# uzh-rpg/rampvo

Measured on AMD Instinct MI355X. Metric: keyframes/sec (BA iters/sec) SingleScale 640x480; ATE vs reference, higher is better.
Workload: dtype f16 (features, MFMA inputs; f32 accumulate, hidden state, BA, geometry: default.yaml MIXED_PRECISION); 1 GPU; BASELINE configs[1]: SingleScale 640x480, 96 patches/frame, default.yaml windows, 2 BA iters/keyframe, steady-state sliding window; edges=38880, edges_end=38880, keyframes_in_window=184, prime_frames=70, clock_warm=480 untimed steady-state steps (0.43 s) before the 5 warm-up steps, frame_pipelining=True, pipeline_gate=signal word stored by the gru launch, full=False

## Files before the change

include/ramp_hip.h:

```cpp
#ifndef RAMP_HIP_H
#define RAMP_HIP_H

#include <stddef.h>
#include <stdint.h>

#ifdef __cplusplus
extern "C" {
#endif

#define RAMP_OK 0
#define RAMP_EINVAL -1
#define RAMP_ELAUNCH -2
#define RAMP_EWORKSPACE -3
#define RAMP_EUNSUPPORTED -4

#define RAMP_F32 0
#define RAMP_F16 1

#define RAMP_CORR_MFMA32 0x40
#define RAMP_CORR_X2 0x80

#define RAMP_NCHW 0
#define RAMP_NHWC 1
#define RAMP_NHWC32 2

const char *ramp_version(void);


int ramp_patchify_fwd(const void *net, const float *coords, void *out, int n, int C, int H,
                      int W, int M, int radius, int bilinear, int dtype, int layout,
                      int out_layout, void *stream);

int ramp_frame_gather(const void *fmap, const void *imap, const float *image, const float *coords, void *gmap,
                      void *imap_p, float *patches, float *clr, unsigned char *colors, int M, int h, int w, int H,
                      int W, int CF, int CI, int dtype, void *stream);

typedef struct {
  const void *fmap;
  int H2, W2;
  float coord_div;
} ramp_corr_level;

int ramp_corr_fwd(const void *fmap1, const ramp_corr_level *levels_host, int nlevels,
                  const float *coords, const int64_t *ii, const int64_t *jj, void *out, int E,
                  int N1, int N2, int C, int P, int radius, int dtype, int layout,
                  void *stream);

int ramp_corr_fwd_ordered(const void *fmap1, const ramp_corr_level *levels_host, int nlevels,
                          const float *coords, const int64_t *ii, const int64_t *jj,
                          const int32_t *order, void *out, int out_row_elems, long mod_ii, long mod_jj, int E,
                          int N1, int N2, int C, int P, int radius, int dtype, int layout, void *stream);

int ramp_pyramid_pack(const void *fmap, void *level1, void *level4, int H, int W, int C, int dtype,
                      void *stream);
int ramp_corr_kplane(void);

size_t ramp_event_stack_workspace_bytes(int bins, int H, int W);
int ramp_event_stack(const int32_t *x, const int32_t *y, const int8_t *p, int N, int bins, int H, int W,
                     int8_t *out_i8, float *out_f32, void *ws, size_t ws_bytes, void *stream);

int ramp_depth_median_fill(const float *patches_src, int F, int M, int P, float *patches_dst, void *stream);
int ramp_depth_median(const float *patches_src, int F, int M, int P, float *out, void *stream);

size_t ramp_event_topk_workspace_bytes(int H, int W);
int ramp_event_topk(const float *events, int bins, int H, int W, int k, int nms_kernel_size, float *coords,
                    int64_t *indices, void *ws, size_t ws_bytes, void *stream);

int ramp_se3_exp(const float *a, float *X, int n, void *stream);
int ramp_se3_log(const float *X, float *a, int n, void *stream);
int ramp_se3_inv(const float *X, float *Y, int n, void *stream);
int ramp_se3_mul(const float *X, const float *Y, float *Z, int n, void *stream);
int ramp_se3_act4(const float *X, const float *p, float *q, int n, void *stream);
int ramp_se3_adj(const float *X, const float *a, float *b, int n, void *stream);
int ramp_se3_adjT(const float *X, const float *a, float *b, int n, void *stream);

int ramp_transform(const float *poses, const float *patches, const float *intrinsics,
                   const int64_t *ii, const int64_t *jj, const int64_t *kk, float *out, int E,
                   int P, int tonly, void *stream);

int ramp_reproject(const float *poses, const float *patches, const float *intrinsics,
                   const int64_t *ii, const int64_t *jj, const int64_t *kk, float *out, int E,
                   int P, void *stream);

int ramp_point_cloud(const float *poses, const float *patches, const float *intrinsics,
                     const int64_t *ix, float *out, int m, int P, void *stream);

int ramp_motionmag(const float *poses, const float *patches, const float *intrinsics,
                   const int64_t *ii, const int64_t *jj, const int64_t *kk, const int32_t *order,
                   const int32_t *seg, const int64_t *ukeys, const int32_t *ngroups, int64_t key_ij,
                   int64_t key_ji, float beta, float *out2, int P, void *stream);

int ramp_motion_model(float *poses, int n, float damping, void *stream);

int ramp_frame_begin(float *poses, int n, int motion, float damping, int64_t *tstamps, int64_t counter,
                     int64_t *index_map, int64_t index_val, float *intrinsics, int copy_k, void *stream);

int ramp_frame_commit(float *poses, int n, int motion, float damping, int64_t *tstamps, int64_t counter,
                      int64_t *index_map, int64_t index_val, float *intrinsics, int copy_k, float *patches_state,
                      int median_frames, int M, int P, float *patches_new, int n_copy, const void *const *src_host,
                      void *const *dst_host, const long *bytes_host, const float *median_dev, void *stream);

int ramp_multi_copy(const void *const *src_host, void *const *dst_host, const long *bytes_host, int n,
                    void *stream);
int ramp_shift_rows(void *const *base_host, const long *row_bytes_host, const int *mod_host, int n, int k,
                    int nrows, void *stream);

size_t ramp_group_by_workspace_bytes(int E);
int ramp_group_by(const int64_t *keys, int E, int64_t key_bound, int32_t *order, int32_t *gid,
                  int32_t *seg_start, int64_t *ukeys, int32_t *ngroups, void *ws,
                  size_t ws_bytes, void *stream);

size_t ramp_neighbors_workspace_bytes(int E);
int ramp_neighbors(const int64_t *kk, const int64_t *jj, int64_t *ix, int64_t *jx, int E,
                   int64_t kk_bound, int64_t jj_bound, void *ws, size_t ws_bytes,
                   void *stream);

int ramp_segment_softmax_sum(const void *fx, const void *gx, const int32_t *order,
                             const int32_t *seg_start, const int32_t *ngroups, void *y, int E,
                             int C, int max_groups, int dtype, void *stream);

size_t ramp_ba_workspace_bytes(int E, int n_poses, int n_patches, int t0, int t1);
int ramp_ba_forward(float *poses, float *patches, const float *intrinsics, const float *target,
                    const float *weight, const float *lmbda, const int64_t *ii,
                    const int64_t *jj, const int64_t *kk, int E, int P, int n_poses,
                    int n_patches, int t0, int t1, int iterations, void *ws, size_t ws_bytes,
                    int32_t *info, void *stream);

size_t ramp_ba_planned_workspace_bytes(int E, int n_poses, int n_patches, int t0, int t1,
                                       int max_patches, int max_pairs);
int ramp_ba_forward_planned(float *poses, float *patches, const float *intrinsics, const float *target,
                            const float *weight, const float *lmbda, const int64_t *ii,
                            const int64_t *jj, const int64_t *kk, int E, int P, int n_poses,
                            int n_patches, int t0, int t1, int iterations, const int32_t *order_k,
                            const int32_t *seg_k, const int32_t *ngroups_k, const int64_t *ukeys_k,
                            int max_patches, const int32_t *order_p, const int32_t *seg_p,
                            const int32_t *ngroups_p, int max_pairs, void *ws, size_t ws_bytes,
                            int32_t *info, void *stream);

size_t ramp_group_by_small_workspace_bytes(int E, int K);
int ramp_group_by_small(const int64_t *a, const int64_t *b, int64_t mul, int64_t sub, int K, int E,
                        int32_t *order, int32_t *gid, int32_t *seg_start, int64_t *ukeys,
                        int32_t *ngroups, int max_groups, void *ws, size_t ws_bytes, void *stream);

int ramp_neighbors_from_groups(const int32_t *order, const int32_t *seg_start, const int32_t *ngroups,
                               const int64_t *jj, int64_t *ix, int64_t *jx, int32_t *kj_order, int E,
                               int max_groups, void *stream);

int ramp_any_nonzero(const float *a, long na, const float *b, long nb, int32_t *flags, void *stream);
int ramp_any_nonzero_blocks(const float *a, long na, const float *b, long nb, int32_t *blockflags, void *stream);
int ramp_any_nonzero_blocks_clear(const float *a, long na, const float *b, long nb, int32_t *blockflags, void *clear,
                                  long clear_bytes, void *stream);

int ramp_lstm_superstate_tiled(const float *ev, const float *im, float *h_ev, float *c_ev, float *h_im,
                               float *c_im, float *ss, const float *wfrag, const int32_t *flags, int HW,
                               int has_state, int has_ss, void *stream);
int ramp_lstm_superstate_blocks(const float *ev, const float *im, float *h_ev, float *c_ev, float *h_im,
                                float *c_im, float *ss, const float *wfrag, const int32_t *blockflags, int nblk, int HW,
                                int has_state, int has_ss, void *stream);

int ramp_ms_lstm_superstate(const float *ev, const float *im, const float *const *weights_host,
                            float *state, int H, int W, int scale, int has_state, int use_im,
                            void *stream);

int ramp_ms_lstm_superstate_mfma(const float *ev, const float *im, const float *wfrag, const float *wsmall, float *state,
                                 void *state16, int H, int W, int scale, int has_state, int use_im, void *stream);

int ramp_conv2d_nhwc(const void *x, const void *wpk, const float *bias, const float *pre_scale,
                     const float *pre_shift, const void *res, void *y, float *stats, int H, int W,
                     int Cin, int Cout, int KH, int KW, int stride, int relu, float out_scale,
                     int dtype, void *stream);

typedef struct ramp_conv_job {
  const void *x, *wpk;
  const float *bias, *pre_scale, *pre_shift;
  const void *res;
  void *y;
  float *stats;
  int32_t Cout, relu;
  float out_scale;
  float act_scale, w_scale;
  void *acc_out;
  const void *acc_in;
  float in_count, in_eps;
  const void *x2;
  int32_t c0;
  const void *skip;
  const void *acc_skip;
  float skip_count, skip_eps;
  int32_t skip_relu;
  void *mat;
} ramp_conv_job;
#define RAMP_IN_ACC_R 8
int ramp_conv2d_nhwc_multi(const ramp_conv_job *jobs, int njobs, int H, int W, int Cin, int KH, int stride,
                           int dtype, void *stream);

#define RAMP_IN_F32 0x10
#define RAMP_CONV_DIRECT 0x20
#define RAMP_CONV_FP8 0x40

#define RAMP_CONV_X3 0x80

int ramp_conv2d_stats_blocks(int H, int W, int Cin, int Cout, int KH, int stride, int dtype);

int ramp_in_stats_finalize(const float *partial, int nblk, int C, float count, float eps, float *scale,
                           float *shift, void *stream);

int ramp_norm_add_relu_f16_acc(const void *y, const void *acc_y, float count_y, float eps_y, const void *skip,
                               const void *acc_skip, float count_skip, float eps_skip, void *out, long n, int C,
                               int skip_relu, void *stream);
int ramp_in_acc_finalize(const void *acc, int C, float count, float eps, float *scale, float *shift, void *stream);

int ramp_affine_relu(const float *x, const float *s, const float *h, float *out, long n, int C,
                     void *stream);

int ramp_affine_relu_f16(const void *x, const float *s, const float *h, void *out, long n, int C,
                         void *stream);
int ramp_norm_add_relu_f16(const void *y, const float *sy, const float *hy, const void *skip,
                           const float *ss, const float *hs, void *out, long n, int C, int skip_relu,
                           void *stream);

int ramp_norm_add_relu(const float *y, const float *sy, const float *hy, const float *skip,
                       const float *ss, const float *hs, float *out, long n, int C, void *stream);

int ramp_upd_row_fuse(const float *A, const int64_t *idxA, const void *B, const void *C, const int64_t *idxB,
                      const int32_t *idxB32, long modB, const int64_t *idxC, const int32_t *idxC32,
                      const float *ln_w, const float *ln_b, float eps, int relu, float *out_f32,
                      void *out_t, int E, int dtype, void *stream);
int ramp_upd_gather_mask(const float *X, const int64_t *idx, void *out, int E, int dtype, void *stream);
int ramp_upd_gated(const float *X, const void *G, const void *R, const float *ln_w, const float *ln_b,
                   float eps, float *out_f32, void *out_t, void *out_relu_t, int E, int dtype,
                   void *stream);
int ramp_upd_heads(const void *hw, const float *coords, float *target, float *weight, float *delta,
                   int E, int P, float wd, float ht, int dtype, void *stream);
int ramp_upd_segment_softmax(const void *fg, const int32_t *order, const int32_t *seg_start,
                             const int32_t *ngroups, void *y, int max_groups, int dtype, void *stream);

int ramp_graph_edit_host(const int64_t *ii, const int64_t *jj, const int64_t *kk, const int64_t *rows_in, int E,
                         int M, int k_remove, int n_after, int removal_window, int64_t *out, int cap,
                         int64_t *ranges );

int ramp_upd_gru(const float *x32, const void *add_t, const int32_t *add_idx, const float *pre_w, const float *pre_b,
                 float pre_eps, const void *const *wp_host, const float *const *bias_host, const float *ln_w,
                 const float *ln_b, float eps, float *out32, void *relu_t, int E, void *stream);
int ramp_upd_gru_heads(const float *x32, const void *add_t, const int32_t *add_idx, const float *pre_w, const float *pre_b,
                       float pre_eps, const void *const *wp_host, const float *const *bias_host, const float *ln_w,
                       const float *ln_b, float eps, float *out32, const void *heads_w, const float *heads_b,
                       const float *coords, float *target, float *weight, int E, int P, float wd, float ht, void *stream);
size_t ramp_upd_mlp_lds_bytes(void);

int ramp_upd_nbr(const float *net_in, const int64_t *idx, const void *wa, const float *ba, const void *wb,
                 const float *bb, float *net_out, void *out_t, int E, void *stream);

int ramp_upd_corr_mlp(const void *corr, int corr_k, const void *w1, const float *b1, const void *w2, const float *b2,
                      const void *w3, const float *b3, const float *ln_w, const float *ln_b, float ln_eps,
                      const float *net, const int64_t *net_map, const void *inp, const int64_t *inp_idx, long inp_mod,
                      const float *norm_w, const float *norm_b, float norm_eps, float *net_out, int E, void *stream);

int ramp_upd_heads_linear(const void *relu_t, const void *heads_w, const float *heads_b, const float *coords,
                          float *target, float *weight, int E, int P, float wd, float ht, void *stream);

int ramp_upd_fg(const float *x32, const void *add_t, const int32_t *add_idx, float *x32_out, const void *wf,
                const float *bf, const void *wg, const float *bg, void *fg, int E, void *stream);

int ramp_upd_linear(const void *x, const void *w_packed, const float *bias, void *y, int rows, const int32_t *rows_dev,
                    void *stream);

size_t ramp_upd_softagg_frag_rows(int E, int max_groups);
int ramp_upd_softagg(const float *x32, const void *add_t, const int32_t *add_idx, const int32_t *order,
                     const int32_t *gid, const void *wf, const float *bf, const void *wg, const float *bg, float *frag,
                     int E, void *stream);
int ramp_upd_softagg_finish(const float *frag, const int32_t *seg_start, const int32_t *ngroups, const void *wh,
                            const float *bh, void *hy, int max_groups, void *stream);

int ramp_x3_corr_mlp(const float *corr, int corr_k, const void *w1, const float *b1, const void *w2, const float *b2,
                     const void *w3, const float *b3, const float *ln_w, const float *ln_b, float ln_eps, const float *net,
                     const int64_t *net_map, const float *inp, const int64_t *inp_idx, long inp_mod, const float *norm_w,
                     const float *norm_b, float norm_eps, float *net_out, int E, void *stream);
int ramp_x3_nbr(const float *net_in, const int64_t *idx, const void *wa, const float *ba, const void *wb, const float *bb,
                float *net_out, int E, void *stream);
// ... 122 lines not shown
```

rampvo_amd/_lib.py:

```python
import ctypes
import os
import subprocess

import torch

_HERE = os.path.dirname(os.path.abspath(__file__))
CSRC = os.path.join(_HERE, "csrc")
LIB_PATH = os.environ.get("RAMP_HIP_LIB") or os.path.join(CSRC, "libramp_hip.so")

RAMP_F32, RAMP_F16 = 0, 1
RAMP_EUNSUPPORTED = -4
RAMP_CONV_FP8 = 0x40
RAMP_IN_F32, RAMP_CONV_DIRECT, RAMP_CORR_MFMA32, RAMP_CORR_X2 = 0x10, 0x20, 0x40, 0x80
RAMP_CONV_X3 = 0x80
RAMP_NCHW, RAMP_NHWC, RAMP_NHWC32 = 0, 1, 2
KPLANE = 32


def kplane(dtype):
    import torch
    return KPLANE if dtype == torch.float16 else KPLANE // 2


def corr_f32_mode():
    import os
    try:
        m = int(os.environ.get("RAMP_CORR_F32_MFMA", "2"))
    except ValueError:
        m = 2
    return m if m in (0, 1, 2) else 2

_ERR = {-1: "RAMP_EINVAL (bad argument)", -2: "RAMP_ELAUNCH (HIP launch/runtime error)",
        -3: "RAMP_EWORKSPACE (workspace too small)", -4: "RAMP_EUNSUPPORTED (size/shape not supported)"}

c_p, c_i, c_i64, c_sz, c_f = ctypes.c_void_p, ctypes.c_int, ctypes.c_int64, ctypes.c_size_t, ctypes.c_float


class CorrLevel(ctypes.Structure):
    _fields_ = [("fmap", c_p), ("H2", c_i), ("W2", c_i), ("coord_div", c_f)]


SIGNATURES = {
    "ramp_version": (ctypes.c_char_p, []),
    "ramp_corr_kplane": (c_i, []),
    "ramp_patchify_fwd": (c_i, [c_p, c_p, c_p] + [c_i] * 10 + [c_p]),
    "ramp_frame_gather": (c_i, [c_p] * 9 + [c_i] * 8 + [c_p]),
    "ramp_corr_fwd": (c_i, [c_p, ctypes.POINTER(CorrLevel), c_i, c_p, c_p, c_p, c_p] + [c_i] * 8 + [c_p]),
    "ramp_ms_lstm_superstate": (c_i, [c_p, c_p, ctypes.POINTER(c_p), c_p, c_i, c_i, c_i, c_i, c_i, c_p]),
    "ramp_ms_lstm_superstate_mfma": (c_i, [c_p] * 6 + [c_i] * 5 + [c_p]),
    "ramp_conv2d_stats_blocks": (c_i, [c_i] * 7),
    "ramp_graph_edit_host": (c_i, [c_p, c_p, c_p, c_p, c_i, c_i, c_i, c_i, c_i, c_p, c_i, c_p]),
    "ramp_event_stack_workspace_bytes": (c_sz, [c_i, c_i, c_i]),
    "ramp_event_stack": (c_i, [c_p, c_p, c_p, c_i, c_i, c_i, c_i, c_p, c_p, c_p, c_sz, c_p]),
    "ramp_depth_median_fill": (c_i, [c_p, c_i, c_i, c_i, c_p, c_p]),
    "ramp_depth_median": (c_i, [c_p, c_i, c_i, c_i, c_p, c_p]),
    "ramp_event_topk_workspace_bytes": (c_sz, [c_i, c_i]),
    "ramp_event_topk": (c_i, [c_p, c_i, c_i, c_i, c_i, c_i, c_p, c_p, c_p, c_sz, c_p]),
    "ramp_pyramid_pack": (c_i, [c_p, c_p, c_p, c_i, c_i, c_i, c_i, c_p]),
    "ramp_corr_fwd_ordered": (c_i, [c_p, ctypes.POINTER(CorrLevel), c_i, c_p, c_p, c_p, c_p, c_p, c_i, ctypes.c_long,
                                    ctypes.c_long] + [c_i] * 8 + [c_p]),
    "ramp_se3_exp": (c_i, [c_p, c_p, c_i, c_p]),
    "ramp_se3_log": (c_i, [c_p, c_p, c_i, c_p]),
    "ramp_se3_inv": (c_i, [c_p, c_p, c_i, c_p]),
    "ramp_se3_mul": (c_i, [c_p, c_p, c_p, c_i, c_p]),
    "ramp_se3_act4": (c_i, [c_p, c_p, c_p, c_i, c_p]),
    "ramp_se3_adj": (c_i, [c_p, c_p, c_p, c_i, c_p]),
    "ramp_se3_adjT": (c_i, [c_p, c_p, c_p, c_i, c_p]),
    "ramp_transform": (c_i, [c_p] * 7 + [c_i, c_i, c_i, c_p]),
    "ramp_reproject": (c_i, [c_p] * 7 + [c_i, c_i, c_p]),
    "ramp_point_cloud": (c_i, [c_p] * 5 + [c_i, c_i, c_p]),
    "ramp_multi_copy": (c_i, [c_p, c_p, c_p, c_i, c_p]),
    "ramp_shift_rows": (c_i, [c_p, c_p, c_p, c_i, c_i, c_i, c_p]),
    "ramp_motionmag": (c_i, [c_p] * 10 + [c_i64, c_i64, c_f, c_p, c_i, c_p]),
    "ramp_motion_model": (c_i, [c_p, c_i, c_f, c_p]),
    "ramp_frame_commit": (c_i, [c_p, c_i, c_i, c_f, c_p, c_i64, c_p, c_i64, c_p, c_i, c_p, c_i, c_i, c_i, c_p, c_i,
                                ctypes.POINTER(c_p), ctypes.POINTER(c_p), ctypes.POINTER(ctypes.c_long), c_p, c_p]),
    "ramp_frame_begin": (c_i, [c_p, c_i, c_i, c_f, c_p, c_i64, c_p, c_i64, c_p, c_i, c_p]),
    "ramp_group_by_workspace_bytes": (c_sz, [c_i]),
    "ramp_group_by": (c_i, [c_p, c_i, c_i64, c_p, c_p, c_p, c_p, c_p, c_p, c_sz, c_p]),
    "ramp_neighbors_workspace_bytes": (c_sz, [c_i]),
    "ramp_neighbors": (c_i, [c_p, c_p, c_p, c_p, c_i, c_i64, c_i64, c_p, c_sz, c_p]),
    "ramp_segment_softmax_sum": (c_i, [c_p] * 6 + [c_i, c_i, c_i, c_i, c_p]),
    "ramp_ba_workspace_bytes": (c_sz, [c_i] * 5),
    "ramp_ba_forward": (c_i, [c_p] * 9 + [c_i] * 7 + [c_p, c_sz, c_p, c_p]),
    "ramp_ba_planned_workspace_bytes": (c_sz, [c_i] * 7),
    "ramp_ba_forward_planned": (c_i, [c_p] * 9 + [c_i] * 7 + [c_p] * 4 + [c_i] + [c_p] * 3 + [c_i, c_p, c_sz, c_p, c_p]),
    "ramp_group_by_small_workspace_bytes": (c_sz, [c_i, c_i]),
    "ramp_group_by_small": (c_i, [c_p, c_p, c_i64, c_i64, c_i, c_i, c_p, c_p, c_p, c_p, c_p, c_i, c_p, c_sz, c_p]),
    "ramp_neighbors_from_groups": (c_i, [c_p] * 7 + [c_i, c_i, c_p]),
    "ramp_any_nonzero": (c_i, [c_p, ctypes.c_long, c_p, ctypes.c_long, c_p, c_p]),
    "ramp_lstm_superstate_tiled": (c_i, [c_p] * 9 + [c_i, c_i, c_i, c_p]),
    "ramp_lstm_superstate_blocks": (c_i, [c_p] * 9 + [c_i, c_i, c_i, c_i, c_p]),
    "ramp_any_nonzero_blocks": (c_i, [c_p, ctypes.c_long, c_p, ctypes.c_long, c_p, c_p]),
    "ramp_any_nonzero_blocks_clear": (c_i, [c_p, ctypes.c_long, c_p, ctypes.c_long, c_p, c_p, ctypes.c_long, c_p]),
    "ramp_conv2d_nhwc": (c_i, [c_p] * 8 + [c_i] * 8 + [c_f, c_i, c_p]),
    "ramp_in_stats_finalize": (c_i, [c_p, c_i, c_i, c_f, c_f, c_p, c_p, c_p]),
    "ramp_affine_relu": (c_i, [c_p, c_p, c_p, c_p, ctypes.c_long, c_i, c_p]),
    "ramp_norm_add_relu": (c_i, [c_p] * 7 + [ctypes.c_long, c_i, c_p]),
    "ramp_affine_relu_f16": (c_i, [c_p, c_p, c_p, c_p, ctypes.c_long, c_i, c_p]),
    "ramp_norm_add_relu_f16": (c_i, [c_p] * 7 + [ctypes.c_long, c_i, c_i, c_p]),
    "ramp_norm_add_relu_f16_acc": (c_i, [c_p, c_p, c_f, c_f, c_p, c_p, c_f, c_f, c_p, ctypes.c_long, c_i, c_i, c_p]),
    "ramp_in_acc_finalize": (c_i, [c_p, c_i, c_f, c_f, c_p, c_p, c_p]),
    "ramp_conv2d_nhwc_multi": (c_i, [c_p, c_i, c_i, c_i, c_i, c_i, c_i, c_i, c_p]),
    "ramp_upd_row_fuse": (c_i, [c_p] * 6 + [ctypes.c_long, c_p, c_p, c_p, c_p, c_f, c_i, c_p, c_p, c_i, c_i, c_p]),
    "ramp_upd_gather_mask": (c_i, [c_p, c_p, c_p, c_i, c_i, c_p]),
    "ramp_upd_gated": (c_i, [c_p] * 5 + [c_f, c_p, c_p, c_p, c_i, c_i, c_p]),
    "ramp_upd_heads": (c_i, [c_p] * 5 + [c_i, c_i, c_f, c_f, c_i, c_p]),
    "ramp_upd_segment_softmax": (c_i, [c_p] * 5 + [c_i, c_i, c_p]),
    "ramp_upd_corr_mlp": (c_i, [c_p, c_i, c_p, c_p, c_p, c_p, c_p, c_p, c_p, c_p, c_f, c_p, c_p, c_p, c_p, ctypes.c_long,
                                c_p, c_p, c_f, c_p, c_i, c_p]),
    "ramp_upd_heads_linear": (c_i, [c_p, c_p, c_p, c_p, c_p, c_p, c_i, c_i, c_f, c_f, c_p]),
    "ramp_upd_fg": (c_i, [c_p] * 9 + [c_i, c_p]),
    "ramp_upd_gru": (c_i, [c_p, c_p, c_p, c_p, c_p, c_f, ctypes.POINTER(c_p), ctypes.POINTER(c_p), c_p, c_p, c_f, c_p,
                           c_p, c_i, c_p]),
    "ramp_upd_gru_heads": (c_i, [c_p, c_p, c_p, c_p, c_p, c_f, ctypes.POINTER(c_p), ctypes.POINTER(c_p), c_p, c_p, c_f, c_p,
                                 c_p, c_p, c_p, c_p, c_p, c_i, c_i, c_f, c_f, c_p]),
    "ramp_upd_mlp_lds_bytes": (c_sz, []),
    "ramp_upd_nbr": (c_i, [c_p] * 8 + [c_i, c_p]),
    "ramp_upd_linear": (c_i, [c_p, c_p, c_p, c_p, c_i, c_p, c_p]),
    "ramp_upd_softagg_frag_rows": (c_sz, [c_i, c_i]),
    "ramp_upd_softagg": (c_i, [c_p] * 10 + [c_i, c_p]),
    "ramp_upd_softagg_finish": (c_i, [c_p] * 6 + [c_i, c_p]),
    "ramp_x3_corr_mlp": (c_i, [c_p, c_i, c_p, c_p, c_p, c_p, c_p, c_p, c_p, c_p, c_f, c_p, c_p, c_p, c_p, ctypes.c_long,
                               c_p, c_p, c_f, c_p, c_i, c_p]),
    "ramp_x3_nbr": (c_i, [c_p] * 7 + [c_i, c_p]),
    "ramp_x3_fg": (c_i, [c_p] * 9 + [c_i, c_p]),
    "ramp_x3_segment_softmax": (c_i, [c_p] * 5 + [c_i, c_p]),
    "ramp_x3_linear": (c_i, [c_p, c_p, c_p, c_p, c_i, c_p, c_p]),
    "ramp_x3_gru": (c_i, [c_p, c_p, c_p, c_p, c_p, c_p, c_p, c_f, ctypes.POINTER(c_p), ctypes.POINTER(c_p), c_p, c_p, c_f,
                          c_p, c_p, c_i, c_p, c_p, c_p, c_p, c_p, c_i, c_f, c_f, c_p]),
    "ramp_track_sizeof": (c_sz, []),
    "ramp_track_plan_workspace_bytes": (c_sz, [c_i, c_i, c_i]),
    "ramp_track_ba_workspace_bytes": (c_sz, [c_i] * 6),
    "ramp_track_plan": (c_i, [c_p, c_i, c_p]),
    "ramp_track_step": (c_i, [c_p, c_i, c_i64, c_i, c_i, c_p, c_p, c_p]),
    "ramp_track_warm": (c_i, [c_p, c_p, c_p]),
    "ramp_stream_delay": (c_i, [c_i, c_p]),
    "ramp_signal_alloc": (c_i, [c_p]),
    "ramp_signal_free": (c_i, [c_p]),
    "ramp_stream_signal": (c_i, [c_p, c_p, ctypes.c_uint32]),
    "ramp_stream_wait_flag": (c_i, [c_p, c_p, ctypes.c_uint32, c_i, c_i, c_p]),
    "ramp_host_device_pointer": (c_i, [c_p, c_p]),
}

_lib = None


def build(force=False, jobs=8):
    cmd = ["make", "-s", "-C", CSRC, "-j%d" % jobs]
    if force:
        cmd.append("-B")
    subprocess.check_call(cmd + ["libramp_hip.so"])
    return LIB_PATH


def register_optional(extra):
    SIGNATURES.update(extra)
    if _lib is not None:
        for name, (res, args) in extra.items():
            fn = getattr(_lib, name)
            fn.restype, fn.argtypes = res, args


def lib():
    global _lib
    if _lib is None:
        if not os.path.exists(LIB_PATH):
            raise RuntimeError(
                "rampvo_amd: %s is missing -- the HIP extension is not built and there is no "
                "CPU fallback (run __graft_entry__.build())" % LIB_PATH)
        l = ctypes.CDLL(LIB_PATH)
        for name, (res, args) in SIGNATURES.items():
            fn = getattr(l, name)
            fn.restype, fn.argtypes = res, args
        if l.ramp_corr_kplane() != KPLANE:
            raise RuntimeError("rampvo_amd: %s packs %d-channel correlation planes, this binding is written for %d "
                               "(rebuild without -DCORR_KPLANE, or set rampvo_amd._lib.KPLANE)" % (LIB_PATH, l.ramp_corr_kplane(), KPLANE))
        _lib = l
    return _lib


def check(rc, what):
    if rc != 0:
        raise RuntimeError("%s failed: %s" % (what, _ERR.get(rc, "status %d" % rc)))


def stream():
    return ctypes.c_void_p(torch._C._cuda_getCurrentRawStream(torch.cuda.current_device()))


def require_cuda(*tensors):
    for t in tensors:
        if t is not None and not t.is_cuda:
            raise RuntimeError("rampvo_amd operators run on the GPU only (got a %s tensor); "
                               "there is no CPU fallback" % t.device)


def dtype_code(t):
    if t.dtype == torch.float32:
        return RAMP_F32
    if t.dtype == torch.float16:
        return RAMP_F16
    raise RuntimeError("unsupported dtype %s (float32 / float16 only)" % t.dtype)


def ptr(t):
    return ctypes.c_void_p(t.data_ptr()) if t is not None else None


_ws_cache = {}
_ws_retired = []
_ws_owner = [None]


class scratch_owner:

    def __init__(self, owner):
        self.owner = owner

    def __enter__(self):
        self.prev, _ws_owner[0] = _ws_owner[0], id(self.owner)

    def __exit__(self, *exc):
        _ws_owner[0] = self.prev


def workspace(nbytes, device, tag="ws"):
    key = (device, torch._C._cuda_getCurrentRawStream(device.index if device.index is not None
                                                      else torch.cuda.current_device()), _ws_owner[0], tag)
    buf = _ws_cache.get(key)
    if buf is None or buf.numel() < nbytes:
        if buf is not None:
            _ws_retired.append(buf)
        buf = torch.empty(max(int(nbytes * 1.25), 1 << 20), dtype=torch.uint8, device=device)
        _ws_cache[key] = buf
    return buf
```

rampvo_amd/csrc/ba.hip:

```cpp
#include "ramp_device.h"
#include <stdlib.h>
#include "ramp_internal.h"

#define BA_REC 32
#define BA_PAIR 160
#define BA_TS 64
#define BA_KB 8

static inline size_t al(size_t x) { return (x + 255) / 256 * 256; }

struct BaEdgeIn {
  const float *poses, *patches, *intr, *target, *weight;
  const int64_t *ii, *jj, *kk;
  int PP, c11, t0, N;
};
__device__ __forceinline__ void ba_edge_compute(const BaEdgeIn &in, int n, float (&r)[BA_REC]) {
  const float fx = in.intr[0], fy = in.intr[1], cx = in.intr[2], cy = in.intr[3];
  int ix = (int)in.ii[n], jx = (int)in.jj[n];
  const long kx = in.kk[n];
  float pi[7], pj[7];
#pragma unroll
  for (int c = 0; c < 7; c++) { pi[c] = in.poses[7 * (size_t)ix + c]; pj[c] = in.poses[7 * (size_t)jx + c]; }
  float Xi[4], Xj[4];
  Xi[0] = (in.patches[((size_t)kx * 3 + 0) * in.PP + in.c11] - cx) / fx;
// ... 629 lines not shown
        for (int k = 0; k < j; k++) x[j] = __builtin_fmaf(-x[k], l[j][k], x[j]);
        x[j] *= li[j];
      }
#pragma unroll
      for (int j = 0; j < 6; j++) A[i * ld + c0 + j] = x[j];
    }
    }
    __syncthreads();
    for (int ii = ty; ii <= m; ii += TG) {
      float ri[6];
#pragma unroll
      for (int k = 0; k < 6; k++) ri[k] = A[(r0 + ii) * ld + c0 + k];
      const int jmax = ii < m - 1 ? ii : m - 1;
      for (int jj = tx; jj <= jmax; jj += TG) {
        const float *rj = A + (r0 + jj) * ld + c0;
        float t = A[(r0 + ii) * ld + r0 + jj];
#pragma unroll
        for (int k = 0; k < 6; k++) t = __builtin_fmaf(-ri[k], rj[k], t);
        A[(r0 + ii) * ld + r0 + jj] = t;
      }
    }
    __syncthreads();
  }
  const bool bad = s_bad != 0;
  if (bad && tid == 0 && info) atomicOr(info, 1);
  if (n6 <= 64) {
    if (tid < 64) {
      float z = tid < n6 ? A[n6 * ld + tid] : 0.0f;
      for (int kb = nb - 1; kb >= 0; kb--) {
        const int c0 = 6 * kb;
        float lk[27], x[6];
#pragma unroll
        for (int q = 0; q < 27; q++) lk[q] = Lk[kb * 28 + q];
#pragma unroll
        for (int j = 0; j < 6; j++) x[j] = __int_as_float(__builtin_amdgcn_readlane(__float_as_int(z), c0 + j));
#pragma unroll
        for (int j = 5; j >= 0; j--) {
#pragma unroll
          for (int k = j + 1; k < 6; k++) x[j] = __builtin_fmaf(-lk[k * (k + 1) / 2 + j], x[k], x[j]);
          x[j] *= lk[21 + j];
        }
        if (tid == 0) {
#pragma unroll
          for (int j = 0; j < 6; j++) xv[c0 + j] = x[j];
        }
        if (tid < c0) {
#pragma unroll
          for (int k = 0; k < 6; k++) z = __builtin_fmaf(-A[(c0 + k) * ld + tid], x[k], z);
        }
      }
    }
    __syncthreads();
  } else
  for (int kb = nb - 1; kb >= 0; kb--) {
    const int c0 = 6 * kb;
    if (tid < 64) {
      float lk[27], x[6];
#pragma unroll
      for (int q = 0; q < 27; q++) lk[q] = Lk[kb * 28 + q];
#pragma unroll
      for (int j = 0; j < 6; j++) x[j] = A[n6 * ld + c0 + j];
#pragma unroll
      for (int j = 5; j >= 0; j--) {
#pragma unroll
        for (int k = j + 1; k < 6; k++) x[j] = __builtin_fmaf(-lk[k * (k + 1) / 2 + j], x[k], x[j]);
        x[j] *= lk[21 + j];
      }
      if (tid == 0) {
#pragma unroll
        for (int j = 0; j < 6; j++) xv[c0 + j] = x[j];
      }
    }
    __syncthreads();
    for (int i = tid; i < c0; i += nt) {
      float t = A[n6 * ld + i];
#pragma unroll
      for (int k = 0; k < 6; k++) t = __builtin_fmaf(-A[(c0 + k) * ld + i], xv[c0 + k], t);
      A[n6 * ld + i] = t;
    }
    __syncthreads();
  }
  __shared__ int s_nf;
  if (tid == 0) s_nf = 0;
  __syncthreads();
  for (int q = tid; q < n6; q += nt)
    if (!(fabsf(xv[q]) <= 3.0e38f)) s_nf = 1;
  __syncthreads();
  const bool drop = bad || s_nf != 0;
  if (!bad && s_nf != 0 && tid == 0 && info) atomicOr(info, 1);
  for (int q = tid; q < n6; q += nt) dX[q] = drop ? 0.0f : xv[q];
}
template <int TG>
__global__ void __launch_bounds__(TG * TG)
    ba_cholb_kernel(const float *__restrict__ S, const float *__restrict__ yv,
                    float *__restrict__ dX, int32_t *__restrict__ info, int n6) {
  extern __shared__ __attribute__((aligned(16))) float sm[];
  const int ld = n6 + 1;
  float *A = sm;
  float *xv = sm + (n6 + 1) * ld;
  float *Lk = xv + n6;
  const int tid = threadIdx.x, nt = TG * TG;
  {
    int r = tid / n6, c = tid - r * n6;
    const int dr = nt / n6, dc = nt - dr * n6;
    for (int q = tid; q < n6 * n6; q += nt) {
      A[r * ld + c] = S[q];
      r += dr; c += dc;
      if (c >= n6) { c -= n6; r++; }
    }
  }
  for (int q = tid; q < n6; q += nt) A[n6 * ld + q] = yv[q];
  ba_cholb_body<TG>(A, xv, Lk, dX, info, n6);
}

__global__ void __launch_bounds__(256)
    ba_retract_kernel(float *__restrict__ poses, float *__restrict__ patches,
                      const float *__restrict__ Erow, const float *__restrict__ Qv,
                      const float *__restrict__ uv, const float *__restrict__ dX,
                      const int64_t *__restrict__ kx, const int32_t *__restrict__ ngroups,
                      int n6, int PP, int t0, int N, int depth_blocks, const int32_t *__restrict__ dyn,
                      int opt_window) {
  if (dyn) {
    const int t1 = dyn[RAMP_DYN_N];
    t0 = max(t1 - opt_window, 1);
    N = min(N, t1 - t0);
  }
  if ((int)blockIdx.x >= depth_blocks) {
    const int i = (blockIdx.x - depth_blocks) * blockDim.x + threadIdx.x;
    if (i >= N) return;
    float *p = poses + 7 * (size_t)(t0 + i);
    float xi[6], to[3] = {p[0], p[1], p[2]}, qo[4] = {p[3], p[4], p[5], p[6]}, tn[3], qn[4];
#pragma unroll
    for (int c = 0; c < 6; c++) xi[c] = dX[6 * i + c];
    fb_retrSE3(xi, to, qo, tn, qn);
    p[0] = tn[0]; p[1] = tn[1]; p[2] = tn[2];
    p[3] = qn[0]; p[4] = qn[1]; p[5] = qn[2]; p[6] = qn[3];
    return;
  }
  const int wave = threadIdx.x / 64, lane = threadIdx.x % 64;
  const int g = blockIdx.x * (blockDim.x / 64) + wave;
  if (g >= *ngroups) return;
  float s = 0.0f;
  for (int a = lane; a < n6; a += 64) s += Erow[(size_t)g * n6 + a] * dX[a];
#pragma unroll
  for (int off = 32; off > 0; off >>= 1) s += __shfl_down(s, off, 64);
  s = __shfl(s, 0, 64);
  const float dz = Qv[g] * (uv[g] - s);
  float *pt = patches + ((size_t)kx[g] * 3 + 2) * PP;
  float dd = pt[0];
  dd = dd + dz;
  dd = (dd > 20) ? 1.0f : dd;
  dd = fmaxf(dd, 1e-4f);
  if (lane < PP) pt[lane] = dd;
}

__global__ void ba_pairkey_kernel(const int64_t *__restrict__ ii, const int64_t *__restrict__ jj,
                                  int64_t *__restrict__ keys, int E, long long np) {
  const int n = blockIdx.x * blockDim.x + threadIdx.x;
  if (n < E) keys[n] = jj[n] * np + ii[n];
}

struct BaWs {
  void *gb; size_t gb_bytes;
  int64_t *pkeys, *kx, *pukeys;
  int32_t *order_k, *seg_k, *order_p, *seg_p, *pair_ij, *counters;
  float *rec, *Erow, *Cv, *uv, *Qv, *pairs, *S_part, *y_part, *S, *yv, *dX;
  int Mu_b, Gp_b, KS, tiles;
};
static size_t ba_carve(void *ws, int E, int n_poses, int n_patches, int N, int own_groups,
                       int max_patches, int max_pairs, BaWs *w) {
  const size_t e = (size_t)(E > 0 ? E : 1);
  const int n6 = 6 * N;
  size_t off = 0;
  char *base = (char *)ws;
  auto take = [&](size_t bytes) { char *p = base ? base + off : nullptr; off += al(bytes); return (void *)p; };
  w->Mu_b = (int)((size_t)n_patches < e ? (size_t)n_patches : e);
  if (max_patches > 0 && max_patches < w->Mu_b) w->Mu_b = max_patches;
  if (w->Mu_b < 1) w->Mu_b = 1;
  const size_t pp = (size_t)n_poses * (size_t)n_poses;
  w->Gp_b = (int)(pp < e ? pp : e);
  if (max_pairs > 0 && max_pairs < w->Gp_b) w->Gp_b = max_pairs;
  if (w->Gp_b < 1) w->Gp_b = 1;
  w->tiles = (n6 + BA_TS - 1) / BA_TS;
  if (w->tiles < 1) w->tiles = 1;
  int ks = 256 / (w->tiles * w->tiles);
  w->KS = ks < 4 ? 4 : (ks > 64 ? 64 : ks);
  w->gb = nullptr; w->gb_bytes = 0;
  w->pkeys = w->kx = w->pukeys = nullptr;
  w->order_k = w->seg_k = w->order_p = w->seg_p = nullptr;
  if (own_groups) {
    w->gb_bytes = ramp_internal_group_by_ws(E);
    w->gb = take(w->gb_bytes);
    w->pkeys = (int64_t *)take(e * 8);
    w->kx = (int64_t *)take(e * 8);
    w->pukeys = (int64_t *)take(e * 8);
    w->order_k = (int32_t *)take(e * 4);
    w->seg_k = (int32_t *)take((e + 1) * 4);
    w->order_p = (int32_t *)take(e * 4);
    w->seg_p = (int32_t *)take((e + 1) * 4);
  }
  w->pair_ij = (int32_t *)take((size_t)w->Gp_b * 8);
  w->counters = (int32_t *)take(64);
  w->rec = (float *)take(e * BA_REC * 4);
  w->Erow = (float *)take((size_t)w->Mu_b * (n6 > 0 ? n6 : 1) * 4);
  w->Cv = (float *)take((size_t)w->Mu_b * 4);
  w->uv = (float *)take((size_t)w->Mu_b * 4);
  w->Qv = (float *)take((size_t)w->Mu_b * 4);
  w->pairs = (float *)take((size_t)w->Gp_b * BA_PAIR * 4);
  w->S_part = (float *)take((size_t)w->KS * (n6 * n6 + 1) * 4);
  w->y_part = (float *)take((size_t)w->KS * (n6 + 1) * 4);
  w->S = (float *)take((size_t)(n6 * n6 + 1) * 4);
  w->yv = (float *)take((size_t)(n6 + 1) * 4);
  w->dX = (float *)take((size_t)(n6 + 1) * 4);
  return off;
}

static int ba_iterate(float *poses, float *patches, const float *intrinsics, const float *target,
                      const float *weight, const float *lmbda, const int64_t *ii, const int64_t *jj,
                      const int64_t *kk, int E, int P, int t0, int t1, int iterations, BaWs &w,
                      const int32_t *order_k, const int32_t *seg_k, const int32_t *nk, const int64_t *kx,
                      const int32_t *order_p, const int32_t *seg_p, const int32_t *np, int32_t *info,
                      hipStream_t st, const int32_t *dyn = nullptr, int opt_window = 0) {
  const int N = t1 - t0, n6 = 6 * N;
  const size_t lds = (size_t)((n6 + 1) * (n6 + 1) + 6 * n6) * sizeof(float);
  const int PP = P * P, c11 = 1 * P + 1;
  if (N > 0 && lds > 64 * 1024) {
    if (hipFuncSetAttribute((const void *)ba_cholb_kernel<32>, hipFuncAttributeMaxDynamicSharedMemorySize, (int)lds) != hipSuccess)
      return RAMP_ELAUNCH;
  }
  const int pthreads = ((n6 + 2 + 63) / 64) * 64;
  if (pthreads > 256) return RAMP_EUNSUPPORTED;
  const int depth_blocks = ramp_cdiv(w.Mu_b, 4);
  const int pose_blocks = N > 0 ? ramp_cdiv(N, 256) : 0;
  BaEdgeIn ein;
  ein.poses = poses; ein.patches = patches; ein.intr = intrinsics; ein.target = target; ein.weight = weight;
  ein.ii = ii; ein.jj = jj; ein.kk = kk; ein.PP = PP; ein.c11 = c11; ein.t0 = t0; ein.N = N;
  const int fuse_edge = 1;
  for (int itr = 0; itr < iterations; itr++) {
    if (N <= 0)
      hipLaunchKernelGGL(ba_edge_kernel, dim3(ramp_cdiv(E, 256)), dim3(256), 0, st, ein, w.rec, E, dyn, opt_window);
    if (N > 0)
      hipLaunchKernelGGL(ba_patch_pair_kernel, dim3(w.Mu_b + w.Gp_b), dim3(256), 0, st, w.Mu_b, w.rec, order_k,
                         seg_k, nk, lmbda, w.Erow, w.Cv, w.uv, w.Qv, n6, order_p, seg_p, np, w.pairs, w.pair_ij, ein,
                         fuse_edge, dyn, opt_window);
    else
      hipLaunchKernelGGL(ba_patch_kernel, dim3(w.Mu_b), dim3(pthreads), 0, st, w.rec, order_k, seg_k, nk,
                         lmbda, w.Erow, w.Cv, w.uv, w.Qv, n6);
    if (N > 0) {
      if (w.tiles == 1 && ramp_cdiv(w.Mu_b, w.KS) <= BA_S1_ROWS)
        hipLaunchKernelGGL(ba_schur1_kernel, dim3(1, 1, w.KS), dim3(256), 0, st, w.Erow, w.Qv, w.uv, nk, w.S_part, w.y_part,
                           n6, w.KS);
      else
        hipLaunchKernelGGL(ba_schur_kernel, dim3(w.tiles, w.tiles, w.KS), dim3(256), 0, st, w.Erow,
                           w.Qv, w.uv, nk, w.S_part, w.y_part, n6, w.KS);
      if (N <= 16)
        hipLaunchKernelGGL(ba_assemble2_kernel, dim3(N, N), dim3(256), 0, st, w.pairs, w.pair_ij, np, w.S_part, w.y_part,
                           w.S, w.yv, n6, w.KS, info);
      else
        hipLaunchKernelGGL(ba_assemble_kernel, dim3(N, ramp_cdiv(6 * n6, 192)), dim3(256), 0, st, w.pairs, w.pair_ij, np,
                           w.S_part, w.y_part, w.S, w.yv, n6, w.KS, info);
      hipLaunchKernelGGL(ba_cholb_kernel<32>, dim3(1), dim3(1024), lds, st, w.S, w.yv, w.dX, info, n6);
    }
    hipLaunchKernelGGL(ba_retract_kernel, dim3(depth_blocks + pose_blocks), dim3(256), 0, st,
                       poses, patches, w.Erow, w.Qv, w.uv, w.dX, kx, nk, n6, PP, t0, N, depth_blocks, dyn, opt_window);
    RAMP_CHECK_LAUNCH();
  }
  return RAMP_OK;
}

static int ba_check_args(int E, int P, int n_poses, int n_patches, int t0, int t1, int iterations) {
  if (E < 0 || P < 2 || n_poses <= 0 || n_patches <= 0 || iterations < 0) return RAMP_EINVAL;
  if (t0 < 0 || t1 < t0 || t1 > n_poses) return RAMP_EINVAL;
  const int n6 = 6 * (t1 - t0);
  if ((size_t)((n6 + 1) * (n6 + 1) + 2 * n6) * sizeof(float) > 160 * 1024) return RAMP_EUNSUPPORTED;
  return RAMP_OK;
}

size_t ramp_i_ba_dyn_ws(int E_cap, int n_poses, int n_patches, int opt_window, int max_patches, int max_pairs) {
  BaWs w;
  return ba_carve(nullptr, E_cap, n_poses, n_patches, opt_window, 0, max_patches, max_pairs, &w);
}
int ramp_i_ba_dyn(float *poses, float *patches, const float *intrinsics, const float *target, const float *weight,
                  const float *lmbda, const int64_t *ii, const int64_t *jj, const int64_t *kk, int E_cap, int P,
                  int n_poses, int n_patches, int opt_window, int iterations, const int32_t *order_k,
                  const int32_t *seg_k, const int32_t *ngroups_k, const int64_t *ukeys_k, int max_patches,
                  const int32_t *order_p, const int32_t *seg_p, const int32_t *ngroups_p, int max_pairs, void *ws,
                  size_t ws_bytes, int32_t *info, const int32_t *dyn, hipStream_t st) {
  if (E_cap <= 0 || opt_window <= 0 || !dyn || !ws) return RAMP_EINVAL;
  int rc = ba_check_args(E_cap, P, n_poses, n_patches, 1, 1 + opt_window, iterations);
  if (rc != RAMP_OK) return rc;
  BaWs w;
  if (ba_carve(ws, E_cap, n_poses, n_patches, opt_window, 0, max_patches, max_pairs, &w) > ws_bytes)
    return RAMP_EWORKSPACE;
  return ba_iterate(poses, patches, intrinsics, target, weight, lmbda, ii, jj, kk, E_cap, P, 1, 1 + opt_window,
                    iterations, w, order_k, seg_k, ngroups_k, ukeys_k, order_p, seg_p, ngroups_p, info, st, dyn,
                    opt_window);
}

extern "C" {

size_t ramp_ba_workspace_bytes(int E, int n_poses, int n_patches, int t0, int t1) {
  BaWs w;
  const int N = t1 - t0 > 0 ? t1 - t0 : 0;
  return ba_carve(nullptr, E, n_poses, n_patches, N, 1, 0, 0, &w);
}

int ramp_ba_forward(float *poses, float *patches, const float *intrinsics, const float *target,
                    const float *weight, const float *lmbda, const int64_t *ii,
                    const int64_t *jj, const int64_t *kk, int E, int P, int n_poses,
                    int n_patches, int t0, int t1, int iterations, void *ws, size_t ws_bytes,
                    int32_t *info, void *stream) {
  int rc = ba_check_args(E, P, n_poses, n_patches, t0, t1, iterations);
  if (rc != RAMP_OK) return rc;
  hipStream_t st = (hipStream_t)stream;
  if (info) (void)hipMemsetAsync(info, 0, sizeof(int32_t), st);
  if (E == 0 || iterations == 0) return RAMP_OK;
  if (!poses || !patches || !intrinsics || !target || !weight || !lmbda || !ii || !jj || !kk || !ws)
    return RAMP_EINVAL;
  const int N = t1 - t0;
  BaWs w;
  if (ba_carve(ws, E, n_poses, n_patches, N, 1, 0, 0, &w) > ws_bytes) return RAMP_EWORKSPACE;
  int32_t *nk = w.counters, *np = w.counters + 1;
  rc = ramp_internal_group_by(kk, E, n_patches, w.order_k, nullptr, w.seg_k, w.kx, nk, w.gb, w.gb_bytes, st);
  if (rc != RAMP_OK) return rc;
  if (N > 0) {
    hipLaunchKernelGGL(ba_pairkey_kernel, dim3(ramp_cdiv(E, 256)), dim3(256), 0, st, ii, jj, w.pkeys, E,
                       (long long)n_poses);
    rc = ramp_internal_group_by(w.pkeys, E, (int64_t)n_poses * n_poses, w.order_p, nullptr, w.seg_p,
                                w.pukeys, np, w.gb, w.gb_bytes, st);
    if (rc != RAMP_OK) return rc;
  }
  return ba_iterate(poses, patches, intrinsics, target, weight, lmbda, ii, jj, kk, E, P, t0, t1, iterations,
                    w, w.order_k, w.seg_k, nk, w.kx, w.order_p, w.seg_p, np, info, st);
}

size_t ramp_ba_planned_workspace_bytes(int E, int n_poses, int n_patches, int t0, int t1,
                                       int max_patches, int max_pairs) {
  BaWs w;
  const int N = t1 - t0 > 0 ? t1 - t0 : 0;
  return ba_carve(nullptr, E, n_poses, n_patches, N, 0, max_patches, max_pairs, &w);
}

int ramp_ba_forward_planned(float *poses, float *patches, const float *intrinsics, const float *target,
                            const float *weight, const float *lmbda, const int64_t *ii,
                            const int64_t *jj, const int64_t *kk, int E, int P, int n_poses,
                            int n_patches, int t0, int t1, int iterations, const int32_t *order_k,
                            const int32_t *seg_k, const int32_t *ngroups_k, const int64_t *ukeys_k,
                            int max_patches, const int32_t *order_p, const int32_t *seg_p,
                            const int32_t *ngroups_p, int max_pairs, void *ws, size_t ws_bytes,
                            int32_t *info, void *stream) {
  int rc = ba_check_args(E, P, n_poses, n_patches, t0, t1, iterations);
  if (rc != RAMP_OK) return rc;
  hipStream_t st = (hipStream_t)stream;
  if (info) (void)hipMemsetAsync(info, 0, sizeof(int32_t), st);
  if (E == 0 || iterations == 0) return RAMP_OK;
  if (!poses || !patches || !intrinsics || !target || !weight || !lmbda || !ii || !jj || !kk || !ws ||
      !order_k || !seg_k || !ngroups_k || !ukeys_k || !order_p || !seg_p || !ngroups_p)
    return RAMP_EINVAL;
  if (max_patches <= 0 || max_pairs <= 0) return RAMP_EINVAL;
  BaWs w;
  if (ba_carve(ws, E, n_poses, n_patches, t1 - t0, 0, max_patches, max_pairs, &w) > ws_bytes)
    return RAMP_EWORKSPACE;
  return ba_iterate(poses, patches, intrinsics, target, weight, lmbda, ii, jj, kk, E, P, t0, t1, iterations,
                    w, order_k, seg_k, ngroups_k, ukeys_k, order_p, seg_p, ngroups_p, info, st);
}

}
```

Measured before the change: 1137 keyframes/s.

## Fuse Cholesky solve and retraction into one redundant-solve BA kernel

```diff
diff --git a/include/ramp_hip.h b/include/ramp_hip.h
--- a/include/ramp_hip.h
+++ b/include/ramp_hip.h
@@ -125,6 +125,11 @@
                     const int64_t *jj, const int64_t *kk, int E, int P, int n_poses,
                     int n_patches, int t0, int t1, int iterations, void *ws, size_t ws_bytes,
                     int32_t *info, void *stream);
+int ramp_ba_forward_seq(float *poses, float *patches, const float *intrinsics, const float *target,
+                        const float *weight, const float *lmbda, const int64_t *ii,
+                        const int64_t *jj, const int64_t *kk, int E, int P, int n_poses,
+                        int n_patches, int t0, int t1, int iterations, void *ws, size_t ws_bytes,
+                        int32_t *info, int separate_solve, float *dX_out, void *stream);
 
 size_t ramp_ba_planned_workspace_bytes(int E, int n_poses, int n_patches, int t0, int t1,
                                        int max_patches, int max_pairs);
diff --git a/rampvo_amd/_lib.py b/rampvo_amd/_lib.py
--- a/rampvo_amd/_lib.py
+++ b/rampvo_amd/_lib.py
@@ -83,6 +83,7 @@
     "ramp_segment_softmax_sum": (c_i, [c_p] * 6 + [c_i, c_i, c_i, c_i, c_p]),
     "ramp_ba_workspace_bytes": (c_sz, [c_i] * 5),
     "ramp_ba_forward": (c_i, [c_p] * 9 + [c_i] * 7 + [c_p, c_sz, c_p, c_p]),
+    "ramp_ba_forward_seq": (c_i, [c_p] * 9 + [c_i] * 7 + [c_p, c_sz, c_p, c_i, c_p, c_p]),
     "ramp_ba_planned_workspace_bytes": (c_sz, [c_i] * 7),
     "ramp_ba_forward_planned": (c_i, [c_p] * 9 + [c_i] * 7 + [c_p] * 4 + [c_i] + [c_p] * 3 + [c_i, c_p, c_sz, c_p, c_p]),
     "ramp_group_by_small_workspace_bytes": (c_sz, [c_i, c_i]),
diff --git a/rampvo_amd/csrc/ba.hip b/rampvo_amd/csrc/ba.hip
--- a/rampvo_amd/csrc/ba.hip
+++ b/rampvo_amd/csrc/ba.hip
@@ -805,6 +805,190 @@
   dd = (dd > 20) ? 1.0f : dd;
   dd = fmaxf(dd, 1e-4f);
   if (lane < PP) pt[lane] = dd;
+}
+
+#define BA_SR_NB 10
+#define BA_SR_PPW 4
+__device__ __forceinline__ void ba_wave_sync() {
+  __builtin_amdgcn_fence(__ATOMIC_RELEASE, "wavefront");
+  __builtin_amdgcn_wave_barrier();
+  __builtin_amdgcn_fence(__ATOMIC_ACQUIRE, "wavefront");
+}
+template <int NB>
+__global__ void __launch_bounds__(256)
+    ba_solve_retract_kernel(const float *__restrict__ S, const float *__restrict__ yv, float *__restrict__ dX,
+                            int32_t *__restrict__ info, float *__restrict__ poses, float *__restrict__ patches,
+                            const float *__restrict__ Erow, const float *__restrict__ Qv, const float *__restrict__ uv,
+                            const int64_t *__restrict__ kx, const int32_t *__restrict__ ngroups, int max_groups, int PP,
+                            int t0, int N, const int32_t *__restrict__ dyn, int opt_window) {
+  static_assert(NB >= 1 && NB <= BA_SR_NB, "6N <= 60");
+  constexpr int n6 = 6 * NB, ld = n6 + 1, nb = NB;
+  __shared__ float A[(n6 + 1) * ld];
+  __shared__ __attribute__((aligned(16))) float s_pan[64][8];
+  __shared__ float Lk[NB * 28];
+  __shared__ float s_x[64];
+  if (dyn) {
+    const int t1 = dyn[RAMP_DYN_N];
+    t0 = max(t1 - opt_window, 1);
+    N = min(N, t1 - t0);
+  }
+  const int tid = threadIdx.x, wave = tid >> 6, lane = tid & 63;
+  const int ng = min(*ngroups, max_groups);
+  const int gw = (blockIdx.x * 4 + wave) * BA_SR_PPW;
+  float e_p[BA_SR_PPW], q_p[BA_SR_PPW], u_p[BA_SR_PPW], d_p[BA_SR_PPW];
+  int64_t k_p[BA_SR_PPW];
+#pragma unroll
+  for (int p = 0; p < BA_SR_PPW; p++) {
+    const int g = gw + p;
+    e_p[p] = 0.0f; q_p[p] = 0.0f; u_p[p] = 0.0f; k_p[p] = 0;
+    if (g < ng) {
+      if (lane < n6) e_p[p] = Erow[(size_t)g * n6 + lane];
+      q_p[p] = Qv[g]; u_p[p] = uv[g]; k_p[p] = kx[g];
+    }
+  }
+#pragma unroll
+  for (int p = 0; p < BA_SR_PPW; p++) d_p[p] = gw + p < ng ? patches[((size_t)k_p[p] * 3 + 2) * PP] : 0.0f;
+  {
+    constexpr int U = (n6 * n6 + 255) / 256;
+    float v[U];
+#pragma unroll
+    for (int u = 0; u < U; u++) { const int q = tid + u * 256; v[u] = q < n6 * n6 ? S[q] : 0.0f; }
+#pragma unroll
+    for (int u = 0; u < U; u++) {
+      const int q = tid + u * 256;
+      if (q < n6 * n6) { const int r = q / n6; A[r * ld + q - r * n6] = v[u]; }
+    }
+    if (tid < n6) A[n6 * ld + tid] = yv[tid];
+  }
+  __syncthreads();
+  if (wave == 0) {
+    float row[n6];
+#pragma unroll
+    for (int c = 0; c < n6; c++) row[c] = lane <= n6 ? A[lane * ld + c] : 0.0f;
+    bool bad = false;
+#pragma unroll
+    for (int kb = 0; kb < nb; kb++) {
+      const int c0 = 6 * kb, r0 = c0 + 6;
+      float l[6][6], li[6];
+#pragma unroll
+      for (int i = 0; i < 6; i++)
+#pragma unroll
+        for (int j = 0; j <= i; j++) l[i][j] = __int_as_float(__builtin_amdgcn_readlane(__float_as_int(row[c0 + j]), c0 + i));
+#pragma unroll
+      for (int j = 0; j < 6; j++) {
+        float d = l[j][j];
+#pragma unroll
+        for (int k = 0; k < j; k++) d = __builtin_fmaf(-l[j][k], l[j][k], d);
+        bad |= !(d > 0.0f);
+        li[j] = __builtin_amdgcn_rsqf(d);
+        l[j][j] = d * li[j];
+#pragma unroll
+        for (int i = j + 1; i < 6; i++) {
+          float t = l[i][j];
+#pragma unroll
+          for (int k = 0; k < j; k++) t = __builtin_fmaf(-l[i][k], l[j][k], t);
+          l[i][j] = t * li[j];
+        }
+      }
+      if (lane == 0) {
+        int q = 0;
+#pragma unroll
+        for (int i = 0; i < 6; i++)
+#pragma unroll
+          for (int j = 0; j <= i; j++) Lk[kb * 28 + q++] = l[i][j];
+#pragma unroll
+        for (int j = 0; j < 6; j++) Lk[kb * 28 + 21 + j] = li[j];
+      }
+      float x[6];
+#pragma unroll
+      for (int j = 0; j < 6; j++) x[j] = row[c0 + j];
+#pragma unroll
+      for (int j = 0; j < 6; j++) {
+#pragma unroll
+        for (int k = 0; k < j; k++) x[j] = __builtin_fmaf(-x[k], l[j][k], x[j]);
+        x[j] *= li[j];
+      }
+#pragma unroll
+      for (int j = 0; j < 6; j++) row[c0 + j] = x[j];
+      ba_wave_sync();
+      *reinterpret_cast<float4 *>(&s_pan[lane][0]) = make_float4(x[0], x[1], x[2], x[3]);
+      *reinterpret_cast<float2 *>(&s_pan[lane][4]) = make_float2(x[4], x[5]);
+      ba_wave_sync();
+#pragma unroll
+      for (int jj = 0; jj < n6 - 6; jj++) {
+        if (r0 + jj < n6) {
+          const float4 a4 = *reinterpret_cast<const float4 *>(&s_pan[r0 + jj][0]);
+          const float2 a2 = *reinterpret_cast<const float2 *>(&s_pan[r0 + jj][4]);
+          const float rj[6] = {a4.x, a4.y, a4.z, a4.w, a2.x, a2.y};
+          float t = row[r0 + jj];
+#pragma unroll
+          for (int k = 0; k < 6; k++) t = __builtin_fmaf(-x[k], rj[k], t);
+          row[r0 + jj] = t;
+        }
+      }
+    }
+#pragma unroll
+    for (int c = 0; c < n6; c++)
+      if (lane <= n6) A[lane * ld + c] = row[c];
+    ba_wave_sync();
+    float z = lane < n6 ? A[n6 * ld + lane] : 0.0f;
+#pragma unroll
+    for (int kb = nb - 1; kb >= 0; kb--) {
+      const int c0 = 6 * kb;
+      float lk[27], x[6];
+#pragma unroll
+      for (int q = 0; q < 27; q++) lk[q] = Lk[kb * 28 + q];
+#pragma unroll
+      for (int j = 0; j < 6; j++) x[j] = __int_as_float(__builtin_amdgcn_readlane(__float_as_int(z), c0 + j));
+#pragma unroll
+      for (int j = 5; j >= 0; j--) {
+#pragma unroll
+        for (int k = j + 1; k < 6; k++) x[j] = __builtin_fmaf(-lk[k * (k + 1) / 2 + j], x[k], x[j]);
+        x[j] *= lk[21 + j];
+      }
+#pragma unroll
+      for (int j = 0; j < 6; j++)
+        if (lane == c0 + j) s_x[lane] = x[j];
+      if (lane < c0) {
+#pragma unroll
+        for (int k = 0; k < 6; k++) z = __builtin_fmaf(-A[(c0 + k) * ld + lane], x[k], z);
+      }
+    }
+    ba_wave_sync();
+    const float xq = lane < n6 ? s_x[lane] : 0.0f;
+    const bool nf = __ballot(lane < n6 && !(fabsf(xq) <= 3.0e38f)) != 0ull;
+    const bool drop = bad || nf;
+    if (lane < n6) {
+      s_x[lane] = drop ? 0.0f : xq;
+      if (blockIdx.x == 0) dX[lane] = drop ? 0.0f : xq;
+    }
+    if (drop && blockIdx.x == 0 && lane == 0 && info) atomicOr(info, 1);
+  }
+  __syncthreads();
+  if (blockIdx.x == 0 && tid < N) {
+    float *p = poses + 7 * (size_t)(t0 + tid);
+    float xi[6], to[3] = {p[0], p[1], p[2]}, qo[4] = {p[3], p[4], p[5], p[6]}, tn[3], qn[4];
+#pragma unroll
+    for (int c = 0; c < 6; c++) xi[c] = s_x[6 * tid + c];
+    fb_retrSE3(xi, to, qo, tn, qn);
+    p[0] = tn[0]; p[1] = tn[1]; p[2] = tn[2];
+    p[3] = qn[0]; p[4] = qn[1]; p[5] = qn[2]; p[6] = qn[3];
+  }
+#pragma unroll
+  for (int p = 0; p < BA_SR_PPW; p++) {
+    if (gw + p >= ng) break;
+    float s = 0.0f;
+    if (lane < n6) s += e_p[p] * s_x[lane];
+#pragma unroll
+    for (int off = 32; off > 0; off >>= 1) s += __shfl_down(s, off, 64);
+    s = __shfl(s, 0, 64);
+    const float dz = q_p[p] * (u_p[p] - s);
+    float dd = d_p[p];
+    dd = dd + dz;
+    dd = (dd > 20) ? 1.0f : dd;
+    dd = fmaxf(dd, 1e-4f);
+    if (lane < PP) patches[((size_t)k_p[p] * 3 + 2) * PP + lane] = dd;
+  }
 }
 
 __global__ void ba_pairkey_kernel(const int64_t *__restrict__ ii, const int64_t *__restrict__ jj,
@@ -873,7 +1057,7 @@
                       const int64_t *kk, int E, int P, int t0, int t1, int iterations, BaWs &w,
                       const int32_t *order_k, const int32_t *seg_k, const int32_t *nk, const int64_t *kx,
                       const int32_t *order_p, const int32_t *seg_p, const int32_t *np, int32_t *info,
-                      hipStream_t st, const int32_t *dyn = nullptr, int opt_window = 0) {
+                      hipStream_t st, const int32_t *dyn = nullptr, int opt_window = 0, int separate_solve = 0) {
   const int N = t1 - t0, n6 = 6 * N;
   const size_t lds = (size_t)((n6 + 1) * (n6 + 1) + 6 * n6) * sizeof(float);
   const int PP = P * P, c11 = 1 * P + 1;
@@ -888,6 +1072,12 @@
   BaEdgeIn ein;
   ein.poses = poses; ein.patches = patches; ein.intr = intrinsics; ein.target = target; ein.weight = weight;
   ein.ii = ii; ein.jj = jj; ein.kk = kk; ein.PP = PP; ein.c11 = c11; ein.t0 = t0; ein.N = N;
+  const bool solve_retract = !separate_solve && N > 0 && n6 <= 6 * BA_SR_NB;
+  const int sr_blocks = ramp_cdiv(w.Mu_b, 4 * BA_SR_PPW);
+  static decltype(&ba_solve_retract_kernel<1>) const sr_kernels[BA_SR_NB] = {
+      ba_solve_retract_kernel<1>, ba_solve_retract_kernel<2>, ba_solve_retract_kernel<3>, ba_solve_retract_kernel<4>,
+      ba_solve_retract_kernel<5>, ba_solve_retract_kernel<6>, ba_solve_retract_kernel<7>, ba_solve_retract_kernel<8>,
+      ba_solve_retract_kernel<9>, ba_solve_retract_kernel<10>};
   const int fuse_edge = 1;
   for (int itr = 0; itr < iterations; itr++) {
     if (N <= 0)
@@ -912,10 +1102,15 @@
       else
         hipLaunchKernelGGL(ba_assemble_kernel, dim3(N, ramp_cdiv(6 * n6, 192)), dim3(256), 0, st, w.pairs, w.pair_ij, np,
                            w.S_part, w.y_part, w.S, w.yv, n6, w.KS, info);
-      hipLaunchKernelGGL(ba_cholb_kernel<32>, dim3(1), dim3(1024), lds, st, w.S, w.yv, w.dX, info, n6);
-    }
-    hipLaunchKernelGGL(ba_retract_kernel, dim3(depth_blocks + pose_blocks), dim3(256), 0, st,
-                       poses, patches, w.Erow, w.Qv, w.uv, w.dX, kx, nk, n6, PP, t0, N, depth_blocks, dyn, opt_window);
+      if (!solve_retract)
+        hipLaunchKernelGGL(ba_cholb_kernel<32>, dim3(1), dim3(1024), lds, st, w.S, w.yv, w.dX, info, n6);
+    }
+    if (solve_retract)
+      hipLaunchKernelGGL(sr_kernels[N - 1], dim3(sr_blocks), dim3(256), 0, st, w.S, w.yv, w.dX, info, poses, patches,
+                         w.Erow, w.Qv, w.uv, kx, nk, w.Mu_b, PP, t0, N, dyn, opt_window);
+    else
+      hipLaunchKernelGGL(ba_retract_kernel, dim3(depth_blocks + pose_blocks), dim3(256), 0, st,
+                         poses, patches, w.Erow, w.Qv, w.uv, w.dX, kx, nk, n6, PP, t0, N, depth_blocks, dyn, opt_window);
     RAMP_CHECK_LAUNCH();
   }
   return RAMP_OK;
@@ -963,6 +1158,15 @@
                     const int64_t *jj, const int64_t *kk, int E, int P, int n_poses,
                     int n_patches, int t0, int t1, int iterations, void *ws, size_t ws_bytes,
                     int32_t *info, void *stream) {
+  return ramp_ba_forward_seq(poses, patches, intrinsics, target, weight, lmbda, ii, jj, kk, E, P, n_poses, n_patches, t0,
+                             t1, iterations, ws, ws_bytes, info, 0, nullptr, stream);
+}
+
+int ramp_ba_forward_seq(float *poses, float *patches, const float *intrinsics, const float *target,
+                        const float *weight, const float *lmbda, const int64_t *ii,
+                        const int64_t *jj, const int64_t *kk, int E, int P, int n_poses,
+                        int n_patches, int t0, int t1, int iterations, void *ws, size_t ws_bytes,
+                        int32_t *info, int separate_solve, float *dX_out, void *stream) {
   int rc = ba_check_args(E, P, n_poses, n_patches, t0, t1, iterations);
   if (rc != RAMP_OK) return rc;
   hipStream_t st = (hipStream_t)stream;
@@ -983,8 +1187,12 @@
                                 w.pukeys, np, w.gb, w.gb_bytes, st);
     if (rc != RAMP_OK) return rc;
   }
-  return ba_iterate(poses, patches, intrinsics, target, weight, lmbda, ii, jj, kk, E, P, t0, t1, iterations,
-                    w, w.order_k, w.seg_k, nk, w.kx, w.order_p, w.seg_p, np, info, st);
+  rc = ba_iterate(poses, patches, intrinsics, target, weight, lmbda, ii, jj, kk, E, P, t0, t1, iterations,
+                  w, w.order_k, w.seg_k, nk, w.kx, w.order_p, w.seg_p, np, info, st, nullptr, 0, separate_solve);
+  if (rc == RAMP_OK && dX_out && N > 0 &&
+      hipMemcpyAsync(dX_out, w.dX, (size_t)6 * N * sizeof(float), hipMemcpyDeviceToDevice, st) != hipSuccess)
+    return RAMP_ELAUNCH;
+  return rc;
 }
 
 size_t ramp_ba_planned_workspace_bytes(int E, int n_poses, int n_patches, int t0, int t1,
```

After: 1123 keyframes/s, median of 2. 0.988x the previous value.
